# gaopinghai/BDE2VID

Measured on AMD Instinct MI355X. Metric: reconstructed frames/sec at 5x240x180 voxels, seq_len=16, higher is better.
Workload: dtype f32 (operands split into two fp16 terms on the matrix cores where conv_sb / lstm_sb / winblock_sb apply: 3 MFMAs per fp32 block, f32 accumulate)

## Files before the change

### bde2vid_amd/csrc/api_model.h

```cpp
#pragma once
namespace bde {

struct DenseLayer {
    int rows = 0, Cin = 0, KS = 1;
    std::vector<float> w, bias, lnsum;
};

struct PackedLayer {
    int Cin = 0, Cout = 0, KS = 1, CK = 8, nchunks = 0, ntiles = 0;
    bool lstm = false;
    long w_off = -1, b_off = -1, s_off = -1;
    long w_sz = 0;
    int G = 1;
    long sb_off = -1, sb_sz = 0;
    long sh_off = -1, sh_sz = 0;
    long sh_unscale_off = -1;
    long split_off(int terms) const { return terms == 2 ? sh_off : sb_off; }
    long split_sz(int terms) const { return terms == 2 ? sh_sz : sb_sz; }
    int sb_chunks = 0;
    long h3_off[2] = {-1, -1};
    long h3_sz[2] = {0, 0};
    mutable int sb_used = 0;
    int G_decide = 0;
};

static PackedLayer group_view(const PackedLayer& pl, int g) {
    PackedLayer v = pl;
    v.G_decide = pl.G;
    v.G = 1;
    v.w_off += g * pl.w_sz;
    if (v.b_off >= 0) v.b_off += (long)g * pl.Cout;
    if (v.s_off >= 0) v.s_off += (long)g * pl.Cout;
    if (v.sb_off >= 0) v.sb_off += g * pl.sb_sz;
    if (v.sh_off >= 0) v.sh_off += g * pl.sh_sz;
    return v;
}

struct Arena {
    std::vector<float> host;
    long alloc(long n) {
        long off = (long)host.size();
        long n4 = (n + 3) / 4 * 4;
        host.resize(off + n4, 0.f);
        return off;
    }
};

struct AttnBlock {
    PackedLayer qkv, proj, fc1, fc2;
    long proj16 = -1, fc1_16 = -1, fc2_16 = -1, qkv16 = -1;
    long projW = -1, fc1W = -1, fc2W = -1, qkvW = -1;
    long projS = -1, fc1S = -1, fc2S = -1, qkvS = -1;
    long projH = -1, fc1H = -1, fc2H = -1, qkvH = -1;
    long unscaleH = -1;
    long projHF = -1, projHF_unscale = -1;
    long fc1N = -1, fc2N = -1, mlpN_unscale = -1;
    long qkvN = -1, qkvN_unscale = -1;
    long kvpad_off = -1;
    long bias_off = -1;
    long biasF_off = -1;
    long biasW_off = -1;
};
struct AttnLevel {
    int depth = 0, C = 0;
    std::vector<AttnBlock> blocks;
    PackedLayer kvall;
    long kvallW = -1;
    long kvallH = -1, kvallH_unscale = -1;
};

struct Workspace {
    int T = 0, B = 0, H = 0, W = 0;
    std::vector<void*> allocs;
    float* ev = nullptr;
    float* head = nullptr;
    float* out = nullptr;
    std::vector<float*> xenc, gx, hseq, cst, merged, mergedT, kvun, kvref, dec, qkv0;
    float *qkv = nullptr, *ao = nullptr, *x1 = nullptr, *hid = nullptr, *xa = nullptr, *xb = nullptr;
    int* tile_count = nullptr;
    std::vector<float*> mergedS, mstats;
    float *xaS = nullptr, *xbS = nullptr, *stA = nullptr, *stB = nullptr;
    float* up = nullptr;
    float* sb = nullptr;
    float* sb2 = nullptr;
    long sb2_bytes = 0;
    std::vector<float*> gur, ghr, gou, gub;
    float *cat = nullptr, *fuse = nullptr;
    float *rbA = nullptr, *rbX[2] = {nullptr, nullptr}, *zero_l = nullptr;
    std::vector<float*> hsk;
    std::vector<float*> hsb, ghb;
    long sb_bytes = 0;
    hipGraphExec_t graph_exec = nullptr;
    int graph_part = 0;
    bool warm = false;
    void release() {
        if (graph_exec) { (void)hipGraphExecDestroy(graph_exec); graph_exec = nullptr; }
        warm = false;
        for (void* p : allocs) (void)hipFree(p);
        allocs.clear();
        ev = head = out = qkv = ao = x1 = hid = xa = xb = up = sb = sb2 = cat = fuse = rbA = rbX[0] = rbX[1] = zero_l = nullptr;
        tile_count = nullptr;
        xaS = xbS = stA = stB = nullptr;
        mergedS.clear(); mstats.clear();
        sb_bytes = sb2_bytes = 0;
        for (auto* v : {&xenc, &gx, &hseq, &cst, &merged, &mergedT, &kvun, &kvref, &dec, &qkv0, &gur, &ghr, &gou, &gub, &hsk, &hsb, &ghb}) v->clear();
        T = B = H = W = 0;
    }
};

}

using namespace bde;

struct bde_model {
    bde_config cfg;
    int L = 0;
    std::map<std::string, std::pair<std::vector<int64_t>, std::vector<float>>> raw;
    bool finalized = false;
    Arena arena;
    float* dev = nullptr;
    long dev_numel = 0;
    PackedLayer head, pred_dummy;
    std::vector<PackedLayer> enc, gx, lstm, lstm8, dec;
    std::vector<PackedLayer> lstm_sb;
    std::vector<PackedLayer> lstm_sbk;
    std::vector<PackedLayer> lstm_sbx;
    std::vector<PackedLayer> gru_ur, gru_o;
    std::vector<PackedLayer> dec_fuse;
    PackedLayer pred_fuse;
    std::vector<PackedLayer> rb1, rb2;
    std::vector<AttnLevel> attn;
    long predw_off = -1, predb_off = -1, zero_off = -1;
    static constexpr int MAX_SLOTS = 4;
    Workspace wslots[MAX_SLOTS];
    int cur = 0;
    Workspace& W() { return wslots[cur]; }
    hipStream_t cap_stream = nullptr;
    int use_graph = 1;
    int pipeline = 1;
    hipStream_t pstream[MAX_SLOTS] = {};
    hipEvent_t pin[MAX_SLOTS] = {}, pout[MAX_SLOTS] = {};
    bool pbusy[MAX_SLOTS] = {};
    hipStream_t last_stream = nullptr;
    long ncalls = 0;
    int device = 0;
    hipStream_t side[MAX_SLOTS + 1] = {};
    std::vector<hipEvent_t> frame_ev[MAX_SLOTS + 1];
    hipEvent_t join_ev[MAX_SLOTS + 1] = {};
    int overlap = 0;
    int eager_cut = 1;
    int overlap_chunk = 4;
    int debug_skip = 0;
    int tok_debug = 0;
    unsigned long long* tok_stamps = nullptr;
    Tuning tune;
    int lstm_hc8 = -1;
    int dir_mask = 3;
    int winblock = 1;
    int winblock_sb = 1;
    int fuse_pred = 1;
    int xcd_remap = 1;
    int head3 = 1;
    int fuse_enc_sb = 1;
    int conv_sb = 1;
    int sb_terms = BDE_DEFAULT_SB_TERMS;
    int lstm_two_streams = 0;
    hipStream_t dir_stream[4] = {};
    hipEvent_t dir_fork[4] = {}, dir_join[4] = {};
    int use_lstm_sbk = 1;
    int wide_kv_sb = 1;
    int wide_fuse_mlp = 1;
    int lstm_fuse_x = 1;
    int lstm_sb_mode = 0;
    long fused_min_tiles = 160;
    unsigned* ovf_dev = nullptr;
    unsigned* ovf_host = nullptr;
    int sb_auto = 1;
    long sb_overflows = 0;
    int sb_latched = 0;
    struct Pending {
        bool on = false;
        hipEvent_t done = nullptr;
        hipStream_t stream = nullptr;
        int T = 0, B = 0, H = 0, W = 0;
        std::vector<float*> images;
    } pend[MAX_SLOTS];
    unsigned* ovf() const { return (ovf_dev && sb_terms == 2) ? ovf_dev + cur : nullptr; }
    bool prof_on = false;
    struct ProfSpan { std::string name; hipEvent_t a, b; };
    std::vector<ProfSpan> prof;
    std::vector<hipEvent_t> prof_pool;

    int cin(int l) const { return cfg.basechannels << l; }
    int cout(int l) const { return cfg.basechannels << (l + 1); }
    const float* P(long off) const { return dev + off; }
    long lstm_sb_off(int l) const { return (size_t)l < lstm_sb.size() ? lstm_sb[l].sb_off : -1; }
    long zero_off_long() const { return zero_off; }
};

namespace bde {

static hipEvent_t prof_event(bde_model* m) {
    hipEvent_t e;
    if (!m->prof_pool.empty()) { e = m->prof_pool.back(); m->prof_pool.pop_back(); return e; }
    if (hipEventCreate(&e) != hipSuccess) return nullptr;
    return e;
}
struct ProfScope {
    bde_model* m; hipStream_t s; hipEvent_t a = nullptr, b = nullptr; const char* name;
    ProfScope(bde_model* m_, const char* n, hipStream_t s_) : m(m_), s(s_), name(n) {
        if (!m->prof_on) return;
        a = prof_event(m); b = prof_event(m);
        if (a) (void)hipEventRecord(a, s);
    }
    ~ProfScope() {
        if (!m->prof_on || !a || !b) return;
        (void)hipEventRecord(b, s);
        m->prof.push_back({name, a, b});
    }
};

static const char* pname(const char* base, int i) {
    static std::map<std::string, std::string> names;
    static std::mutex mu;
    const std::string k = std::string(base) + std::to_string(i);
// ... 6 lines not shown
```

### bde2vid_amd/csrc/api_schedule.h

```cpp
#pragma once
namespace bde {

struct ConvCall {
    const PackedLayer* pl = nullptr;
    const float* in = nullptr;
    float* out = nullptr;
    const float* res1 = nullptr;
    const float* res2 = nullptr;
    int N = 1, Hs = 0, Ws = 0;
    int stride = 1;
    int act = ACT_NONE;
    long in_gs = 0, out_gs = 0;
    int mask_w = 0, mask_pt = 0, mask_pl = 0;
    int cout_rows = -1;
    const float* pred_head = nullptr;
    float* pred_out = nullptr;
    float* out_sb = nullptr;
    long out_sb_gs = 0;
    bool in_sb = false;
    int decide_N = 0;
};

static bool conv_takes_sb(const bde_model* m, const PackedLayer& pl, int stride, int N, int Hs, int Ws) {
    const int pad = pl.KS / 2;
// ... 1051 lines not shown
}

static int run_bottleneck_level(bde_model* m, int l, int T, int B, int h, int w, hipStream_t s) {
    const bde_config& c = m->cfg;
    Workspace& ws = m->W();
    const int C = m->cout(l), nb = c.num_res_blocks;
    const long fs = (long)B * C * h * w;
    for (int t = 0; t < T; ++t) {
        ProfScope ps(m, pname("bottleneck", l), s);
        const int f = t + c.buffer_index[0];
        float* mt = ws.merged[l] + (long)t * fs;
        const float* x = (f < 0 || f >= T) ? ws.zero_l : ws.merged[l] + (long)f * fs;
        if (nb == 0) { BDE_TRY(add2(x, mt, mt, fs, s)); continue; }
        for (int k = 0; k < nb; ++k) {
            ConvCall c1;
            c1.pl = &m->rb1[k]; c1.in = x; c1.out = ws.rbA; c1.N = B; c1.Hs = h; c1.Ws = w; c1.act = ACT_RELU;
            BDE_TRY(run_conv(m, c1, s));
            const bool last = k == nb - 1;
            ConvCall c2;
            c2.pl = &m->rb2[k]; c2.in = ws.rbA; c2.N = B; c2.Hs = h; c2.Ws = w; c2.act = ACT_NONE;
            c2.res1 = x;
            c2.res2 = last ? mt : nullptr;
            c2.out = last ? mt : ws.rbX[k & 1];
            BDE_TRY(run_conv(m, c2, s));
            x = c2.out;
        }
    }
    return BDE_OK;
}

enum { PART_ALL = 0, PART_MAIN = 1, PART_TAIL = 2, PART_PRE = 3 };

static int run_decoder(bde_model* m, int j, const float* in, const float* skip, float* out, int N, int Hs, int Ws,
                       hipStream_t s, const float* pred_head = nullptr, float* pred_out = nullptr, int part = PART_ALL, int decide_N = 0) {
    const PackedLayer& pl = m->dec[j];
    Workspace& ws = m->W();
    if (decide_N <= 0) decide_N = N;
    const bool to_sb = m->fuse_enc_sb && (!pred_out || pl.Cout <= 32) && conv_takes_sb(m, pl, 1, decide_N, 2 * Hs, 2 * Ws) && ws.sb &&
                       split_bf16_bytes(N, pl.Cin, 4L * Hs * Ws) <= ws.sb_bytes;
    if (part != PART_TAIL) {
        ProfScope ps(m, pname("dec_up", j), s);
        if (to_sb) BDE_TRY(upsample2x_sum_split(in, skip, ws.sb, N, pl.Cin, Hs, Ws, m->sb_terms, m->ovf(), s));
        else BDE_TRY(upsample2x_sum(in, skip, ws.up, Hs, Ws, (long)N * pl.Cin, s));
    }
    if (part == PART_MAIN) return BDE_OK;
    ConvCall d;
    d.pl = &pl;
    d.in = to_sb ? ws.sb : ws.up;
    d.in_sb = to_sb;
    d.out = out;
    d.N = N;
    d.Hs = 2 * Hs;
    d.Ws = 2 * Ws;
    d.act = ACT_RELU6;
    d.pred_head = pred_head;
    d.pred_out = pred_out;
    d.decide_N = decide_N;
    ProfScope ps(m, pname("dec_conv", j), s);
    return run_conv(m, d, s);
}

static int check_dims(const bde_model* m, int T, int B, int H, int W) {
    const bde_config& c = m->cfg;
    BDE_REQUIRE(m->finalized, "weights are not finalized");
    BDE_REQUIRE(T >= 1 && B >= 1, "T=%d B=%d", T, B);
    const int mult = 1 << c.num_encoders;
    BDE_REQUIRE(H > 0 && W > 0 && H % mult == 0 && W % mult == 0, "H=%d W=%d must be multiples of %d", H, W, mult);
    for (int l = 0; l < c.num_encoders; ++l)
        if (c.depths[l] > 0)
            BDE_REQUIRE((H >> (l + 1)) >= 7 && (W >> (l + 1)) >= 7,
                        "feature map %dx%d at attention level %d is smaller than the 7x7 window (the reference "
                        "raises there too)", H >> (l + 1), W >> (l + 1), l);
    return BDE_OK;
}

static int forward_on(bde_model* m, const float* const* events, int T, int B, int H, int W, float* const* images,
                      hipStream_t s);

static int pipeline_stream(int slot, hipStream_t* out) {
    static hipStream_t pool[BDE_MAX_DEVICES][bde_model::MAX_SLOTS] = {};
    int d = 0;
    BDE_HIP(hipGetDevice(&d));
    BDE_REQUIRE(d >= 0 && d < BDE_MAX_DEVICES, "device %d", d);
    if (!pool[d][slot]) BDE_HIP(hipStreamCreateWithFlags(&pool[d][slot], hipStreamNonBlocking));
    *out = pool[d][slot];
    return BDE_OK;
}

static int note_overflow_readback(bde_model* m, hipStream_t s) {
    bde_model::Pending& p = m->pend[m->cur];
    if (!p.done) BDE_HIP(hipEventCreateWithFlags(&p.done, hipEventDisableTiming));
    BDE_HIP(hipMemcpyAsync(m->ovf_host + m->cur, m->ovf_dev + m->cur, sizeof(unsigned), hipMemcpyDeviceToHost, s));
    BDE_HIP(hipEventRecord(p.done, s));
    return BDE_OK;
}
static void note_pending(bde_model* m, int slot, hipStream_t s, int T, int B, int H, int W, float* const* images) {
    bde_model::Pending& p = m->pend[slot];
    p.on = true; p.stream = s; p.T = T; p.B = B; p.H = H; p.W = W;
    p.images.assign(images, images + T);
}
static int settle_overflow(bde_model* m) {
    bool flagged[bde_model::MAX_SLOTS] = {};
    int nflag = 0;
    for (int i = 0; i < bde_model::MAX_SLOTS; ++i) {
        bde_model::Pending& p = m->pend[i];
        if (!p.on) continue;
        BDE_HIP(hipEventSynchronize(p.done));
        if (m->ovf_host[i] != 0) { flagged[i] = true; ++nflag; }
    }
    if (nflag == 0) {
        for (auto& p : m->pend) p.on = false;
        return BDE_OK;
    }
    m->sb_overflows += nflag;
    for (int i = 0; i < bde_model::MAX_SLOTS; ++i) m->ovf_host[i] = 0;
    if (!m->sb_auto) {
        for (auto& p : m->pend) p.on = false;
        return fail(BDE_ERR_RANGE, "%d forward(s): an activation reached 65520, beyond the two fp16 terms of the default operand format "
                    "(csrc/split.h); the frames of those calls are not valid.  set_tuning(\"sb_terms\", 3) or \"sb_auto\" = 1", nflag);
    }
    for (int i = 0; i < bde_model::MAX_SLOTS; ++i)
        if (m->pend[i].on) BDE_HIP(hipStreamSynchronize(m->pend[i].stream));
    struct Redo { int slot; float* ev; long ev_fs; };
    std::vector<Redo> redo;
    for (int i = 0; i < bde_model::MAX_SLOTS; ++i) {
        if (!flagged[i]) continue;
        const bde_model::Pending& p = m->pend[i];
        const long ev_fs = (long)p.B * m->cfg.num_bins * p.H * p.W;
        float* ev = nullptr;
        BDE_HIP(hipMalloc((void**)&ev, sizeof(float) * ev_fs * p.T));
        BDE_HIP(hipMemcpy(ev, m->wslots[i].ev, sizeof(float) * ev_fs * p.T, hipMemcpyDeviceToDevice));
        redo.push_back({i, ev, ev_fs});
    }
    for (auto& w : m->wslots) w.release();
    m->sb_terms = 3;
    m->sb_latched = 1;
    int st = BDE_OK;
    for (const Redo& r : redo) {
        bde_model::Pending p = m->pend[r.slot];
        std::vector<const float*> evp(p.T);
        for (int t = 0; t < p.T; ++t) evp[t] = r.ev + (long)t * r.ev_fs;
        m->cur = r.slot;
        if (st == BDE_OK) st = forward_on(m, evp.data(), p.T, p.B, p.H, p.W, p.images.data(), p.stream);
        (void)hipStreamSynchronize(p.stream);
        (void)hipFree(r.ev);
    }
    m->cur = 0;
    for (auto& p : m->pend) p.on = false;
    return st;
}

static int forward_impl(bde_model* m, const float* const* events, int T, int B, int H, int W, float* const* images,
                        hipStream_t user) {
    if (m->pipeline < 2) {
        for (const auto& p : m->pend) if (p.on) { BDE_TRY(settle_overflow(m)); break; }
        m->cur = 0;
        BDE_TRY(forward_on(m, events, T, B, H, W, images, user));
        if (m->ovf() == nullptr) return BDE_OK;
        note_pending(m, 0, user, T, B, H, W, images);
        return settle_overflow(m);
    }
    const int slot = (int)(m->ncalls++ % m->pipeline);
    if (m->pend[slot].on) BDE_TRY(settle_overflow(m));
    if (!m->pstream[slot]) {
        BDE_TRY(pipeline_stream(slot, &m->pstream[slot]));
        BDE_HIP(hipEventCreateWithFlags(&m->pin[slot], hipEventDisableTiming));
        BDE_HIP(hipEventCreateWithFlags(&m->pout[slot], hipEventDisableTiming));
    }
    m->cur = slot;
    BDE_HIP(hipEventRecord(m->pin[slot], user));
    BDE_HIP(hipStreamWaitEvent(m->pstream[slot], m->pin[slot], 0));
    m->last_stream = m->pstream[slot];
    const int st = forward_on(m, events, T, B, H, W, images, m->pstream[slot]);
    if (st == BDE_OK && m->ovf() != nullptr) note_pending(m, slot, m->pstream[slot], T, B, H, W, images);
    BDE_HIP(hipEventRecord(m->pout[slot], m->pstream[slot]));
    m->pbusy[slot] = true;
    m->cur = 0;
    return st;
}

static int forward_body(bde_model* m, int T, int B, int H, int W, hipStream_t s, int part);
static bool side_decode_on(const bde_model* m, int T);

static int forward_on(bde_model* m, const float* const* events, int T, int B, int H, int W, float* const* images,
                      hipStream_t s) {
    BDE_TRY(check_dims(m, T, B, H, W));
    BDE_TRY(ensure_workspace(m, T, B, H, W));
    Workspace& ws = m->W();
    const long ev_fs = (long)B * m->cfg.num_bins * H * W, img_fs = (long)B * H * W;
    BDE_TRY(copy_frames(events, ws.ev, T, ev_fs, 0, s));
    ProfScope whole(m, "forward", s);
    const bool guard = m->ovf() != nullptr;
    const bool cut = guard && m->eager_cut && m->pipeline < 2 && m->fuse_enc_sb && !(m->debug_skip & (8 | 16)) && !m->prof_on;
    const int part_main = cut ? PART_MAIN : PART_ALL;
    if (guard) BDE_HIP(hipMemsetAsync(m->ovf(), 0, sizeof(unsigned), s));
    if (cut) BDE_TRY(forward_body(m, T, B, H, W, s, PART_PRE));
    const bool can_graph = m->use_graph && ws.warm && !side_decode_on(m, T);
    if (ws.graph_exec && ws.graph_part != part_main) { (void)hipGraphExecDestroy(ws.graph_exec); ws.graph_exec = nullptr; }
    if (can_graph && !ws.graph_exec) {
        if (!m->cap_stream) BDE_HIP(hipStreamCreateWithFlags(&m->cap_stream, hipStreamNonBlocking));
        hipGraph_t graph = nullptr;
        BDE_HIP(hipStreamBeginCapture(m->cap_stream, hipStreamCaptureModeRelaxed));
        const int st = forward_body(m, T, B, H, W, m->cap_stream, part_main);
        ws.graph_part = part_main;
        const hipError_t e = hipStreamEndCapture(m->cap_stream, &graph);
        hipError_t ei = hipSuccess;
        if (st == BDE_OK && e == hipSuccess) ei = hipGraphInstantiate(&ws.graph_exec, graph, nullptr, nullptr, 0);
        if (graph) (void)hipGraphDestroy(graph);
        if (st != BDE_OK || e != hipSuccess || ei != hipSuccess) {
            (void)hipGetLastError();
            ws.graph_exec = nullptr;
            m->use_graph = 0;
        }
    }
    if (m->use_graph && can_graph && ws.graph_exec) {
        BDE_HIP(hipGraphLaunch(ws.graph_exec, s));
    } else {
        BDE_TRY(forward_body(m, T, B, H, W, s, part_main));
        ws.warm = true;
    }
    if (guard && cut) BDE_TRY(note_overflow_readback(m, s));
    if (cut) BDE_TRY(forward_body(m, T, B, H, W, s, PART_TAIL));
    if (guard && !cut) BDE_TRY(note_overflow_readback(m, s));
    BDE_TRY(copy_frames(images, ws.out, T, img_fs, 1, s));
    return BDE_OK;
}

static int decode_frames(bde_model* mm, int f0, int nf, int T_, int B_, int H_, int W_, hipStream_t st, int part = PART_ALL) {
    Workspace& w = mm->W();
    const int L_ = mm->L;
    const float* x = w.merged[L_ - 1] + (long)f0 * mm->cout(L_ - 1) * (H_ >> L_) * (W_ >> L_);
    for (int j = 0; j < L_; ++j) {
        const int l = L_ - 1 - j;
        const long in_fs = (long)mm->cout(l) * (H_ >> (l + 1)) * (W_ >> (l + 1));
        const long out_fs = (long)mm->cin(l) * (H_ >> l) * (W_ >> l);
        const bool lastj = j == L_ - 1;
        const int jpart = part == PART_ALL ? PART_ALL : (lastj ? part : (part == PART_MAIN ? PART_ALL : -1));
        if (jpart >= 0) {
            ProfScope ps(mm, "decoder", st);
            const bool fuse = lastj && pred_fusable(mm);
            const float* skip = w.merged[l] + (long)f0 * in_fs;
            if (mm->cfg.skip_concat) {
                if (jpart != PART_TAIL)
                    BDE_TRY(run_concat_fuse(mm, mm->dec_fuse[j], skip, x, nf, mm->cout(l), (long)(H_ >> (l + 1)) * (W_ >> (l + 1)), st));
                x = w.fuse;
                skip = nullptr;
            }
            BDE_TRY(run_decoder(mm, j, x, skip, w.dec[j] + (long)f0 * out_fs, nf,
                                H_ >> (l + 1), W_ >> (l + 1), st,
                                fuse ? w.head + (long)f0 * mm->cfg.basechannels * H_ * W_ : nullptr,
                                fuse ? w.out + (long)f0 * H_ * W_ : nullptr, jpart, T_ * B_));
        }
        x = w.dec[j] + (long)f0 * out_fs;
    }
    if (part == PART_MAIN) return BDE_OK;
    if (pred_fusable(mm)) return BDE_OK;
    const long total = (long)nf * H_ * W_;
    long blocks = std::min<long>(cdivl(total, 256), 4096);
    ProfScope ps(mm, "pred", st);
    const float* hd = w.head + (long)f0 * mm->cfg.basechannels * H_ * W_;
    if (mm->cfg.skip_concat) {
        BDE_TRY(run_concat_fuse(mm, mm->pred_fuse, x, hd, nf, mm->cfg.basechannels, (long)H_ * W_, st));
        x = w.fuse;
        hd = nullptr;
    }
    hipLaunchKernelGGL(pred_kernel, dim3((unsigned)blocks), dim3(256), 0, st, x,
                       hd, mm->P(mm->predw_off),
                       mm->P(mm->predb_off), w.out + (long)f0 * H_ * W_, mm->cfg.basechannels, (long)H_ * W_, total,
                       mm->cfg.activation);
    BDE_HIP(hipGetLastError());
    return BDE_OK;
}

static bool side_decode_on(const bde_model* m, int T) {
    const bde_config& c = m->cfg;
    const bool plain_flags = c.use_rc && c.recurrent_type == 0 && !c.skip_concat && c.depths[c.num_encoders - 1] > 0;
    return m->overlap != 0 && plain_flags && !(m->debug_skip & (2 | 8)) && !m->prof_on && T > m->overlap_chunk;
}

static int forward_body(bde_model* m, int T, int B, int H, int W, hipStream_t s, int part) {
    const bde_config& c = m->cfg;
    Workspace& ws = m->W();
    const int L = c.num_encoders;
    const long TB = (long)T * B;
    const bool side_decode = side_decode_on(m, T);
    const int last_chunk_t0 = side_decode ? (T - 1) / m->overlap_chunk * m->overlap_chunk : 0;
    const int tail_f0 = last_chunk_t0 * B, tail_nf = (int)TB - tail_f0;
    if (part == PART_TAIL) return (m->debug_skip & 8) ? BDE_OK : decode_frames(m, tail_f0, tail_nf, T, B, H, W, s, PART_TAIL);
    if (part != PART_MAIN) {
        { ProfScope ps(m, "head", s); BDE_TRY(run_head_conv(m, ws.ev, ws.head, (int)TB, H, W, s)); }
        if (!(m->debug_skip & 16)) BDE_TRY(run_enc_gx(m, 0, ws.head, 0, (int)TB, T, B, H, W, s));
        if (part == PART_PRE) return BDE_OK;
    }
    struct SideCtx { int T, B, H, W, chunk, slot; hipStream_t main, side; };
    static auto decode_fn = decode_frames;
    const int slot = (m->cap_stream && s == m->cap_stream) ? bde_model::MAX_SLOTS : m->cur;
    if (side_decode && !m->side[slot]) {
        int lo = 0, hi = 0;
        BDE_HIP(hipDeviceGetStreamPriorityRange(&lo, &hi));
        BDE_HIP(hipStreamCreateWithPriority(&m->side[slot], hipStreamNonBlocking, lo));
        BDE_HIP(hipEventCreateWithFlags(&m->join_ev[slot], hipEventDisableTiming));
    }
    while (side_decode && (int)m->frame_ev[slot].size() < T) {
        hipEvent_t e;
        BDE_HIP(hipEventCreateWithFlags(&e, hipEventDisableTiming));
        m->frame_ev[slot].push_back(e);
    }
    const float* target = ws.head;
    bool decoded = false;
    for (int l = 0; l < L; ++l) {
        const int Hl = H >> l, Wl = W >> l, h = Hl / 2, w = Wl / 2, C = m->cout(l);
        BDE_TRY(run_recurrent_level(m, l, target, T, B, Hl, Wl, s, l == 0));
        const long n = TB * C * h * w;
        { ProfScope ps(m, pname("merge", l), s); BDE_TRY(add2(ws.hseq[l], ws.hseq[l] + n, ws.merged[l], n, s)); }
        if (c.depths[l] > 0 && !(m->debug_skip & (l == 0 ? 1 : 2))) {
            static const char* names[BDE_MAX_LEVELS] = {"attn0", "attn1", "attn2", "attn3", "attn4", "attn5", "attn6", "attn7"};
            ProfScope ps(m, names[l], s);
            SideCtx sc{T, B, H, W, m->overlap_chunk, slot, s, m->side[slot]};
            FrameDoneFn fn = nullptr;
            const bool fork = side_decode && l == L - 1;
            if (fork) {
                fn = [](bde_model* mm, int t, void* vp) -> int {
                    SideCtx* q = (SideCtx*)vp;
                    const int done = t + 1;
                    if (done % q->chunk != 0 || done > (q->T - 1) / q->chunk * q->chunk) return BDE_OK;
                    const int t0 = done - q->chunk;
                    BDE_HIP(hipEventRecord(mm->frame_ev[q->slot][t], q->main));
                    BDE_HIP(hipStreamWaitEvent(q->side, mm->frame_ev[q->slot][t], 0));
                    return decode_fn(mm, t0 * q->B, q->chunk * q->B, q->T, q->B, q->H, q->W, q->side, PART_ALL);
                };
            }
            BDE_TRY(run_attention_level(m, l, T, B, h, w, s, fn, &sc));
            if (fork) {
                BDE_HIP(hipEventRecord(m->join_ev[slot], m->side[slot]));
                BDE_HIP(hipStreamWaitEvent(s, m->join_ev[slot], 0));
                decoded = true;
            }
        }
        if (l == L - 1 && c.depths[l] == 0) BDE_TRY(run_bottleneck_level(m, l, T, B, h, w, s));
        target = ws.merged[l];
    }
    if (m->debug_skip & 8) return BDE_OK;
    const int dpart = part == PART_MAIN ? PART_MAIN : PART_ALL;
    if (decoded) return decode_frames(m, tail_f0, tail_nf, T, B, H, W, s, dpart);
    return decode_frames(m, 0, (int)TB, T, B, H, W, s, dpart);
}

static int validate_config(const bde_config* c) {
    BDE_REQUIRE(c != nullptr, "null config");
    BDE_REQUIRE(c->num_encoders >= 1 && c->num_encoders <= BDE_MAX_LEVELS, "num_encoders=%d", c->num_encoders);
    BDE_REQUIRE(c->num_bins >= 1 && c->basechannels >= 1, "num_bins=%d basechannels=%d", c->num_bins, c->basechannels);
    BDE_REQUIRE(c->ks == 3 || c->ks == 5, "ks=%d (3 or 5)", c->ks);
    BDE_REQUIRE(c->frame_num >= 1 && c->frame_num <= BDE_MAX_FRAMES, "frame_num=%d", c->frame_num);
    BDE_REQUIRE(c->q_idx >= 0 && c->q_idx < c->frame_num, "q_idx=%d", c->q_idx);
    BDE_REQUIRE(c->buffer_index[c->q_idx] == 0, "buffer_index[q_idx] must be 0 (the query frame is the current frame)");
    BDE_REQUIRE(c->activation == 0 || c->activation == 1, "activation=%d", c->activation);
    BDE_REQUIRE(c->recurrent_type == 0 || c->recurrent_type == 1, "recurrent_type=%d (0 ConvLSTM, 1 ConvGRU)", c->recurrent_type);
    BDE_REQUIRE(c->use_rc == 0 || c->use_rc == 1, "use_rc=%d", c->use_rc);
    BDE_REQUIRE(c->skip_concat == 0 || c->skip_concat == 1, "skip_concat=%d", c->skip_concat);
    BDE_REQUIRE(c->norm >= 0 && c->norm <= 2, "norm=%d (0 none, 1 BN, 2 IN)", c->norm);
    BDE_REQUIRE(c->num_res_blocks >= 0 && c->num_res_blocks <= 64, "num_res_blocks=%d", c->num_res_blocks);
    for (int l = 0; l < c->num_encoders; ++l) {
        BDE_REQUIRE(c->depths[l] >= 0, "depths[%d]=%d", l, c->depths[l]);
        if (c->depths[l] > 0) {
            const int C = c->basechannels << (l + 1);
            BDE_REQUIRE(c->num_heads >= 1 && C % c->num_heads == 0, "C=%d not divisible by %d heads", C, c->num_heads);
            const int hd = C / c->num_heads;
            BDE_REQUIRE(hd == 1 || hd == 2 || hd == 4 || hd == 8 || hd == 16 || hd == 32, "head_dim=%d not built", hd);
        }
    }
    return BDE_OK;
}


}
```

### bde2vid_amd/csrc/bde_api.hip

```cpp
#include <hip/hip_runtime.h>

#include <algorithm>
#include <cmath>
#include <cstdlib>
#include <map>
#include <memory>
#include <mutex>
#include <string>
#include <vector>

#include "../../include/bde2vid.h"
#include "attn.h"
#include "common.h"
#include "conv_mfma.h"
#include "pw_gemm.h"
#include "token_fused.h"
#include "lstm16.h"
#include "lstm_sb.h"
#include "winblock.h"
#include "winblock_sb.h"
#include "wideblock.h"
#include "wide_mlp.h"
#include "wide_core.h"
#include "conv_vec.h"
#include "conv_sb.h"
#include "voxel.h"
#include "metrics.h"

namespace bde {

int conv_tu_occupancy(const char* kernel);

std::string& last_error_ref() {
    static thread_local std::string e;
    return e;
}
int fail(int code, const char* fmt, ...) {
    char buf[1024];
    va_list ap;
    va_start(ap, fmt);
    vsnprintf(buf, sizeof buf, fmt, ap);
    va_end(ap);
    last_error_ref() = buf;
    return code;
}
}

#include "api_elementwise.h"
#include "api_model.h"
#include "api_pack.h"
#include "api_schedule.h"


extern "C" {
#pragma GCC visibility push(default)

const char* bde_last_error(void) { return last_error_ref().c_str(); }
int bde_abi_version(void) { return 4; }

int bde_create(const bde_config* cfg, bde_model** out) {
    BDE_REQUIRE(out != nullptr, "null out");
    BDE_TRY(validate_config(cfg));
    bde_model* m = new bde_model();
    if (const char* e = getenv("BDE_SB_TERMS")) {
        if (e[0] == '3' && e[1] == 0) m->sb_terms = 3;
        else if (e[0] == '2' && e[1] == 0) m->sb_terms = 2;
    }
    m->cfg = *cfg;
    m->L = cfg->num_encoders;
    *out = m;
    return BDE_OK;
}

void bde_destroy(bde_model* m) {
    if (!m) return;
    for (auto& w : m->wslots) w.release();
    if (m->cap_stream) (void)hipStreamDestroy(m->cap_stream);
    for (int i = 0; i < bde_model::MAX_SLOTS; ++i) {
        if (m->pin[i]) (void)hipEventDestroy(m->pin[i]);
        if (m->pout[i]) (void)hipEventDestroy(m->pout[i]);
    }
    if (m->dev) (void)hipFree(m->dev);
    if (m->ovf_dev) (void)hipFree(m->ovf_dev);
    if (m->ovf_host) (void)hipHostFree(m->ovf_host);
    for (auto& p : m->pend) if (p.done) (void)hipEventDestroy(p.done);
    for (int i = 0; i < 4; ++i) {
        if (m->dir_fork[i]) (void)hipEventDestroy(m->dir_fork[i]);
        if (m->dir_join[i]) (void)hipEventDestroy(m->dir_join[i]);
        if (m->dir_stream[i]) (void)hipStreamDestroy(m->dir_stream[i]);
    }
    for (auto& sp : m->prof) { (void)hipEventDestroy(sp.a); (void)hipEventDestroy(sp.b); }
    for (auto e : m->prof_pool) (void)hipEventDestroy(e);
    for (int i = 0; i <= bde_model::MAX_SLOTS; ++i) {
        for (auto e : m->frame_ev[i]) (void)hipEventDestroy(e);
        if (m->join_ev[i]) (void)hipEventDestroy(m->join_ev[i]);
        if (m->side[i]) (void)hipStreamDestroy(m->side[i]);
    }
    delete m;
}

int bde_load_weight(bde_model* m, const char* key, const float* data, const int64_t* shape, int32_t ndim) {
    BDE_REQUIRE(m && key && data && shape && ndim >= 1 && ndim <= 8, "bad argument");
    int64_t n = 1;
    std::vector<int64_t> sh(shape, shape + ndim);
    for (auto v : sh) {
        BDE_REQUIRE(v >= 1, "weight '%s' has a non-positive dimension", key);
        n *= v;
    }
    m->raw[key] = {sh, std::vector<float>(data, data + n)};
    m->finalized = false;
    return BDE_OK;
}

int bde_finalize_weights(bde_model* m) {
    BDE_REQUIRE(m != nullptr, "null model");
    BDE_TRY(build_packed(m));
    BDE_HIP(hipGetDevice(&m->device));
    return upload(m);
}

int bde_alloc_packed(bde_model* m) {
    BDE_REQUIRE(m != nullptr, "null model");
    const bde_config& c = m->cfg;
    auto put = [&](const std::string& k, std::vector<int64_t> sh) {
        int64_t n = 1;
        for (auto v : sh) n *= v;
        m->raw[GP + k] = {sh, std::vector<float>((size_t)n, 0.f)};
    };
    const int L = c.num_encoders, ks = c.ks, bc = c.basechannels;
    auto put_convlayer = [&](const std::string& p, int cout, int cin) {
        put(p + "conv2d.weight", {cout, cin, ks, ks});
        if (c.norm != 1) put(p + "conv2d.bias", {cout});
        if (c.norm == 1) { put(p + "norm_layer.weight", {cout}); put(p + "norm_layer.bias", {cout}); }
        if (c.norm) { put(p + "norm_layer.running_mean", {cout}); put(p + "norm_layer.running_var", {cout}); }
    };
    put_convlayer("head.", bc, c.num_bins);
    const char* dirs[2] = {"forward_encoder", "backward_encoder"};
    for (int d = 0; d < 2; ++d)
        for (int l = 0; l < L; ++l) {
            std::string p = std::string(dirs[d]) + "." + std::to_string(l) + ".";
            const int ci = bc << l, co = bc << (l + 1);
            if (!c.use_rc) { put_convlayer(p, co, ci); continue; }
            put_convlayer(p + "conv.", co, ci);
            if (c.recurrent_type == 1) {
                for (const char* gate : {"update_gate", "reset_gate", "out_gate"}) {
                    put(p + "recurrent_block." + gate + ".weight", {co, 2 * co, 3, 3});
                    put(p + "recurrent_block." + gate + ".bias", {co});
                }
            } else {
                put(p + "recurrent_block.Gates.weight", {4 * co, 2 * co, 3, 3});
                put(p + "recurrent_block.Gates.bias", {4 * co});
            }
        }
    if (c.depths[L - 1] == 0)
        for (int k = 0; k < c.num_res_blocks; ++k) {
            std::string p = "feat_attns." + std::to_string(L - 1) + "." + std::to_string(1 + k) + ".";
            const int C = bc << L;
            put(p + "conv1.weight", {C, C, 3, 3}); put(p + "conv1.bias", {C});
            put(p + "conv2.weight", {C, C, 3, 3}); put(p + "conv2.bias", {C});
        }
    const int tbl = (2 * c.frame_num - 1) * 169;
    for (int l = 0; l < L; ++l) {
        const int C = bc << (l + 1);
// ... 62 lines not shown
    TuningScope ts(&m->tune);
    int T, B, H, W;
    m->cur = 0;
    BDE_TRY(split_dims(m, &T, &B, &H, &W));
    Workspace& ws = m->W();
    const float* target = level == 0 ? ws.head : ws.merged[level - 1];
    m->dir_mask = 1 << direction;
    const int st = run_recurrent_level(m, level, target, T, B, H >> level, W >> level, (hipStream_t)stream);
    m->dir_mask = 3;
    return st;
}

int bde_split_attend(bde_model* m, int32_t level, void* stream) {
    BDE_REQUIRE(m && level >= 0 && level < m->L, "bad argument");
    TuningScope ts(&m->tune);
    hipStream_t s = (hipStream_t)stream;
    int T, B, H, W;
    m->cur = 0;
    BDE_TRY(split_dims(m, &T, &B, &H, &W));
    Workspace& ws = m->W();
    const int h = H >> (level + 1), w = W >> (level + 1);
    const long n = (long)T * B * m->cout(level) * h * w;
    BDE_TRY(add2(ws.hseq[level], ws.hseq[level] + n, ws.merged[level], n, s));
    if (m->cfg.depths[level] > 0) return run_attention_level(m, level, T, B, h, w, s);
    if (level == m->L - 1) return run_bottleneck_level(m, level, T, B, h, w, s);
    return BDE_OK;
}

int bde_split_decode(bde_model* m, float* const* images, void* stream) {
    BDE_REQUIRE(m && images, "null argument");
    TuningScope ts(&m->tune);
    hipStream_t s = (hipStream_t)stream;
    int T, B, H, W;
    m->cur = 0;
    BDE_TRY(split_dims(m, &T, &B, &H, &W));
    for (int t = 0; t < T; ++t) BDE_REQUIRE(images[t], "null frame pointer at t=%d", t);
    BDE_TRY(decode_frames(m, 0, T * B, T, B, H, W, s));
    BDE_TRY(copy_frames(images, m->W().out, T, (long)B * H * W, 1, s));
    if (m->ovf()) {
        unsigned v = 0;
        BDE_HIP(hipMemcpyAsync(m->ovf_host, m->ovf(), sizeof v, hipMemcpyDeviceToHost, s));
        BDE_HIP(hipStreamSynchronize(s));
        v = m->ovf_host[0];
        m->ovf_host[0] = 0;
        if (v) {
            BDE_HIP(hipMemset(m->ovf(), 0, sizeof v));
            ++m->sb_overflows;
            return fail(BDE_ERR_RANGE, "split forward: an activation reached 65520, beyond the two fp16 terms of the default operand "
                        "format (csrc/split.h); set_tuning(\"sb_terms\", 3) on both ranks and run it again");
        }
    }
    return BDE_OK;
}

int bde_split_buffer(bde_model* m, const char* what, int32_t level, int32_t direction, float** ptr, int64_t* numel) {
    BDE_REQUIRE(m && what && ptr && numel && level >= 0 && level < m->L, "bad argument");
    int T, B, H, W;
    m->cur = 0;
    BDE_TRY(split_dims(m, &T, &B, &H, &W));
    Workspace& ws = m->W();
    const long n = (long)T * B * m->cout(level) * (long)(H >> (level + 1)) * (W >> (level + 1));
    const std::string k(what);
    if (k == "hidden") {
        BDE_REQUIRE(direction == 0 || direction == 1, "direction=%d", direction);
        *ptr = ws.hseq[level] + (long)direction * n;
    } else if (k == "level_out") {
        *ptr = ws.merged[level];
    } else {
        return fail(BDE_ERR_ARG, "unknown split buffer '%s' (hidden | level_out)", what);
    }
    *numel = n;
    return BDE_OK;
}

int bde_wait_outputs(bde_model* m, void* stream) {
    BDE_REQUIRE(m != nullptr, "null model");
    TuningScope ts(&m->tune);
    const int st = settle_overflow(m);
    for (int i = 0; i < bde_model::MAX_SLOTS; ++i)
        if (m->pbusy[i]) {
            BDE_HIP(hipStreamWaitEvent((hipStream_t)stream, m->pout[i], 0));
            m->pbusy[i] = false;
        }
    return st;
}

int bde_set_tuning(bde_model* m, const char* key, int64_t value) {
    BDE_REQUIRE(m && key, "null argument");
    if (std::string(key) == "graph") { m->use_graph = (int)value; return BDE_OK; }
    if (std::string(key) == "pipeline") {
        BDE_REQUIRE(value >= 1 && value <= bde_model::MAX_SLOTS, "pipeline depth must be 1..%d", bde_model::MAX_SLOTS);
        m->pipeline = (int)value;
        return BDE_OK;
    }
    if (std::string(key) == "sb_auto") {
        BDE_REQUIRE(value == 0 || value == 1, "sb_auto: 0 (an overflow of the two-term format fails the call) or 1 (recompute with three terms)");
        m->sb_auto = (int)value;
        return BDE_OK;
    }
    {
        TuningScope ts(&m->tune);
        for (const auto& p : m->pend) if (p.on) { BDE_TRY(settle_overflow(m)); break; }
    }
    for (auto& w : m->wslots)
        if (w.graph_exec) { (void)hipGraphExecDestroy(w.graph_exec); w.graph_exec = nullptr; }
    if (std::string(key) == "lstm_hc8") { m->lstm_hc8 = (int)value; return BDE_OK; }
    if (std::string(key) == "winblock") {
        if (m->winblock != (int)value)
            for (auto& w : m->wslots) w.release();
        m->winblock = (int)value;
        return BDE_OK;
    }
    if (std::string(key) == "winblock_sb") { m->winblock_sb = (int)value; return BDE_OK; }
    if (std::string(key) == "wide_kv_sb" || std::string(key) == "wide_fuse_mlp") {
        int& v = std::string(key) == "wide_kv_sb" ? m->wide_kv_sb : m->wide_fuse_mlp;
        if (v != (int)value)
            for (auto& w : m->wslots) w.release();
        v = (int)value;
        return BDE_OK;
    }
    if (std::string(key) == "conv_sb") {
        if (m->conv_sb != (int)value)
            for (auto& w : m->wslots) w.release();
        m->conv_sb = (int)value;
        return BDE_OK;
    }
    if (std::string(key) == "sb_terms") {
        BDE_REQUIRE(value == 2 || value == 3, "sb_terms: 2 (two fp16 terms) or 3 (three bf16 terms)");
        if (m->sb_terms != (int)value)
            for (auto& w : m->wslots) w.release();
        m->sb_terms = (int)value;
        m->sb_latched = 0;
        return BDE_OK;
    }
    if (std::string(key) == "fuse_enc_sb") { m->fuse_enc_sb = (int)value; return BDE_OK; }
    if (std::string(key) == "head3") { m->head3 = (int)value; return BDE_OK; }
    if (std::string(key) == "xcd_remap") { m->xcd_remap = (int)value; return BDE_OK; }
    if (std::string(key) == "lstm_two_streams") { m->lstm_two_streams = (int)value; return BDE_OK; }
    if (std::string(key) == "lstm_fuse_x") {
        if (m->lstm_fuse_x != (int)value)
            for (auto& w : m->wslots) w.release();
        m->lstm_fuse_x = (int)value;
        return BDE_OK;
    }
    if (std::string(key) == "lstm_sbk") {
        if (m->use_lstm_sbk != (int)value)
            for (auto& w : m->wslots) w.release();
        m->use_lstm_sbk = (int)value;
        return BDE_OK;
    }
    if (std::string(key) == "lstm_sb") {
        if (m->lstm_sb_mode != (int)value)
            for (auto& w : m->wslots) w.release();
        m->lstm_sb_mode = (int)value;
        return BDE_OK;
    }
    if (std::string(key) == "fuse_pred") { m->fuse_pred = (int)value; return BDE_OK; }
    if (std::string(key) == "fused_min_tiles") { m->fused_min_tiles = value; return BDE_OK; }
    if (std::string(key) == "pw_batched") { m->tune.pw_batched = (int)value; return BDE_OK; }
    if (std::string(key) == "pw_force") { m->tune.pw_force = (int)value; return BDE_OK; }
    if (std::string(key) == "conv_nt") { m->tune.conv_nt = (int)value; return BDE_OK; }
    if (std::string(key) == "conv_vec") { m->tune.conv_vec = (int)value; return BDE_OK; }
    if (std::string(key) == "lstm_shape") { m->tune.lstm_shape = (int)value; return BDE_OK; }
    if (std::string(key) == "tok_npt") { m->tune.tok_npt = (int)value; return BDE_OK; }
    if (std::string(key) == "tok_debug") { m->tok_debug = (int)value; return BDE_OK; }
    if (std::string(key) == "overlap") { m->overlap = (int)value; return BDE_OK; }
    if (std::string(key) == "eager_cut") { m->eager_cut = (int)value; return BDE_OK; }
    if (std::string(key) == "debug_skip") { m->debug_skip = (int)value; return BDE_OK; }
    if (std::string(key) == "overlap_chunk") { m->overlap_chunk = std::max<int>(1, (int)value); return BDE_OK; }
    return fail(BDE_ERR_ARG, "unknown tuning key '%s'", key);
}

int bde_get_info(const bde_model* m, const char* key, int64_t* value) {
    BDE_REQUIRE(m && key && value, "null argument");
    const std::string k(key);
    if (k == "debug_skip") *value = m->debug_skip;
    else if (k == "graph") *value = m->use_graph;
    else if (k == "graphs_live") {
        int64_t n = 0;
        for (const auto& w : m->wslots) n += w.graph_exec != nullptr;
        *value = n;
    } else if (k == "pipeline") *value = m->pipeline;
    else if (k == "last_stream") *value = (int64_t)(uintptr_t)m->last_stream;
    else if (k == "device") *value = m->device;
    else if (k == "winblock") *value = m->winblock;
    else if (k == "winblock_sb") *value = m->winblock_sb;
    else if (k == "conv_sb") *value = m->conv_sb;
    else if (k == "head3") *value = m->head3;
    else if (k == "lstm_sb") *value = m->lstm_sb_mode;
    else if (k == "lstm_sbk") *value = m->use_lstm_sbk;
    else if (k == "lstm_fuse_x") *value = m->lstm_fuse_x;
    else if (k == "wide_kv_sb") *value = m->wide_kv_sb;
    else if (k == "wide_fuse_mlp") *value = m->wide_fuse_mlp;
    else if (k == "wide_core2") {
        int64_t v = 0;
        for (int l = 0; l < m->L; ++l) v |= wide_ok(m, l) && split_chain_ok(m, l);
        *value = v;
    }
    else if (k == "sb_terms") *value = m->sb_terms;
    else if (k == "sb_auto") *value = m->sb_auto;
    else if (k == "sb_overflows") *value = m->sb_overflows;
    else if (k == "sb_latched") *value = m->sb_latched;
    else if (k == "sb_overflow_word") {
        unsigned v = 0;
        if (m->ovf_dev) {
            BDE_HIP(hipDeviceSynchronize());
            BDE_HIP(hipMemcpy(&v, m->ovf_dev, sizeof v, hipMemcpyDeviceToHost));
            BDE_HIP(hipMemset(m->ovf_dev, 0, sizeof v));
        }
        *value = v;
    }
    else if (k == "packed_numel") *value = m->dev_numel;
    else if (k == "sb_head") *value = m->head.sb_used;
    else if (k.compare(0, 3, "sb_") == 0 && k.size() >= 5 && k.back() >= '0' && k.back() - '0' < m->L) {
        const int i = k.back() - '0';
        const std::string what = k.substr(3, k.size() - 4);
        if (what == "enc") *value = m->enc[i].sb_used;
        else if (what == "gx") *value = m->gx[i].sb_used;
        else if (what == "dec") *value = m->dec[i].sb_used;
        else if (what == "lstm") *value = (size_t)i < m->lstm_sbk.size() ? m->lstm_sbk[i].sb_used : 0;
        else return fail(BDE_ERR_ARG, "unknown info key '%s'", key);
    }
    else return fail(BDE_ERR_ARG, "unknown info key '%s'", key);
    return BDE_OK;
}

int bde_debug_token_stamps(bde_model* m, int64_t* host_out, int32_t n) {
    BDE_REQUIRE(m != nullptr, "null model");
    if (!m->tok_stamps) {
        BDE_HIP(hipMalloc((void**)&m->tok_stamps, sizeof(unsigned long long) * 64 * 4 * 8));
        BDE_HIP(hipMemset(m->tok_stamps, 0, sizeof(unsigned long long) * 64 * 4 * 8));
        BDE_HIP(hipMemset(m->tok_stamps + 2046, 0xff, sizeof(unsigned long long)));
    }
    if (host_out) {
        BDE_HIP(hipDeviceSynchronize());
        BDE_HIP(hipMemcpy(host_out, m->tok_stamps, sizeof(int64_t) * std::min(n, 64 * 4 * 8), hipMemcpyDeviceToHost));
        BDE_HIP(hipMemset(m->tok_stamps + 2046, 0xff, sizeof(unsigned long long)));
        BDE_HIP(hipMemset(m->tok_stamps + 2047, 0, sizeof(unsigned long long)));
    }
    return BDE_OK;
}

int bde_debug_conv_shape(int32_t ks, int32_t stride, int32_t cout, int32_t in_h, int32_t in_w, int32_t* row_tiles) {
    const int pad = ks / 2;
    const int Ho = (in_h + 2 * pad - ks) / stride + 1, Wo = (in_w + 2 * pad - ks) / stride + 1;
    const int terms = BDE_DEFAULT_SB_TERMS;
    const int shape = conv_sb_pick(ks, stride, cout, in_w, Ho, Wo, terms);
    if (row_tiles) {
        if (shape == SB_32x256T) *row_tiles = -conv_sb_tile_cols(256, Ho, Wo);
        else if (shape == SB_64x128T) *row_tiles = -conv_sb_tile_cols(128, Ho, Wo);
        else *row_tiles = shape == SB_NONE ? 0 : conv_sb_tile_mode(ks, stride, shape == SB_128x64 ? 64 : 128, in_w, Ho, Wo, terms);
    }
    return shape;
}

float bde_debug_split(const float* x, int64_t n, int32_t terms, float scale, uint16_t* out) {
    if (!x || !out || n <= 0 || (terms != 2 && terms != 3)) return 0.f;
    for (int64_t i = 0; i < n; ++i) {
        unsigned short t[3];
        split_terms(x[i], terms, scale, t);
        for (int k = 0; k < terms; ++k) out[i * terms + k] = t[k];
    }
    return terms == 2 ? sb_weight_scale(x, (long)n) : 1.f;
}

// ... 325 lines not shown
```

Measured before the change: 1931.

## Stagger pipelined slots with lead events and stream priorities

Adds a stagger point: each pipelined call records an event partway through the level loop (default after level 0's attention), and the next slot's stream waits on it. Consecutive frames then start offset rather than all contending at once. Odd pipeline slots get created with a different stream priority, and overflow settling now waits only on the slot being reused instead of all pending work. The intent is to reduce contention between concurrent slots while still overlapping them; the cost is added cross-stream dependencies that could serialize work, and graphs are rebuilt when the stagger point changes.

```diff
diff --git a/bde2vid_amd/csrc/api_model.h b/bde2vid_amd/csrc/api_model.h
--- a/bde2vid_amd/csrc/api_model.h
+++ b/bde2vid_amd/csrc/api_model.h
@@ -92,6 +92,7 @@
     long sb_bytes = 0;
     hipGraphExec_t graph_exec = nullptr;
     int graph_part = 0;
+    int graph_lead = 0;
     bool warm = false;
     void release() {
         if (graph_exec) { (void)hipGraphExecDestroy(graph_exec); graph_exec = nullptr; }
@@ -141,6 +142,9 @@
     hipStream_t pstream[MAX_SLOTS] = {};
     hipEvent_t pin[MAX_SLOTS] = {}, pout[MAX_SLOTS] = {};
     bool pbusy[MAX_SLOTS] = {};
+    int stagger = 2;
+    hipEvent_t lead[MAX_SLOTS] = {};
+    int lead_from = -1;
     hipStream_t last_stream = nullptr;
     long ncalls = 0;
     int device = 0;
diff --git a/bde2vid_amd/csrc/api_schedule.h b/bde2vid_amd/csrc/api_schedule.h
--- a/bde2vid_amd/csrc/api_schedule.h
+++ b/bde2vid_amd/csrc/api_schedule.h
@@ -1157,7 +1157,15 @@
     int d = 0;
     BDE_HIP(hipGetDevice(&d));
     BDE_REQUIRE(d >= 0 && d < BDE_MAX_DEVICES, "device %d", d);
-    if (!pool[d][slot]) BDE_HIP(hipStreamCreateWithFlags(&pool[d][slot], hipStreamNonBlocking));
+    if (!pool[d][slot]) {
+        if (slot & 1) {
+            int lo = 0, hi = 0;
+            BDE_HIP(hipDeviceGetStreamPriorityRange(&lo, &hi));
+            BDE_HIP(hipStreamCreateWithPriority(&pool[d][slot], hipStreamNonBlocking, lo));
+        } else {
+            BDE_HIP(hipStreamCreateWithFlags(&pool[d][slot], hipStreamNonBlocking));
+        }
+    }
     *out = pool[d][slot];
     return BDE_OK;
 }
@@ -1225,28 +1233,43 @@
     return st;
 }
 
+static int settle_slot(bde_model* m, int slot) {
+    bde_model::Pending& p = m->pend[slot];
+    if (!p.on) return BDE_OK;
+    BDE_HIP(hipEventSynchronize(p.done));
+    if (m->ovf_host[slot] != 0) return settle_overflow(m);
+    p.on = false;
+    return BDE_OK;
+}
+
+static int lead_point(const bde_model* m) { return m->pipeline >= 2 ? m->stagger : 0; }
+
 static int forward_impl(bde_model* m, const float* const* events, int T, int B, int H, int W, float* const* images,
                         hipStream_t user) {
     if (m->pipeline < 2) {
         for (const auto& p : m->pend) if (p.on) { BDE_TRY(settle_overflow(m)); break; }
         m->cur = 0;
+        m->lead_from = -1;
         BDE_TRY(forward_on(m, events, T, B, H, W, images, user));
         if (m->ovf() == nullptr) return BDE_OK;
         note_pending(m, 0, user, T, B, H, W, images);
         return settle_overflow(m);
     }
     const int slot = (int)(m->ncalls++ % m->pipeline);
-    if (m->pend[slot].on) BDE_TRY(settle_overflow(m));
+    BDE_TRY(settle_slot(m, slot));
     if (!m->pstream[slot]) {
         BDE_TRY(pipeline_stream(slot, &m->pstream[slot]));
         BDE_HIP(hipEventCreateWithFlags(&m->pin[slot], hipEventDisableTiming));
         BDE_HIP(hipEventCreateWithFlags(&m->pout[slot], hipEventDisableTiming));
+        BDE_HIP(hipEventCreateWithFlags(&m->lead[slot], hipEventDisableTiming));
     }
     m->cur = slot;
     BDE_HIP(hipEventRecord(m->pin[slot], user));
     BDE_HIP(hipStreamWaitEvent(m->pstream[slot], m->pin[slot], 0));
+    if (m->lead_from >= 0 && m->lead_from != slot) BDE_HIP(hipStreamWaitEvent(m->pstream[slot], m->lead[m->lead_from], 0));
     m->last_stream = m->pstream[slot];
     const int st = forward_on(m, events, T, B, H, W, images, m->pstream[slot]);
+    m->lead_from = (st == BDE_OK && lead_point(m) > 0) ? slot : -1;
     if (st == BDE_OK && m->ovf() != nullptr) note_pending(m, slot, m->pstream[slot], T, B, H, W, images);
     BDE_HIP(hipEventRecord(m->pout[slot], m->pstream[slot]));
     m->pbusy[slot] = true;
@@ -1271,13 +1294,17 @@
     if (guard) BDE_HIP(hipMemsetAsync(m->ovf(), 0, sizeof(unsigned), s));
     if (cut) BDE_TRY(forward_body(m, T, B, H, W, s, PART_PRE));
     const bool can_graph = m->use_graph && ws.warm && !side_decode_on(m, T);
-    if (ws.graph_exec && ws.graph_part != part_main) { (void)hipGraphExecDestroy(ws.graph_exec); ws.graph_exec = nullptr; }
+    if (ws.graph_exec && (ws.graph_part != part_main || ws.graph_lead != lead_point(m))) {
+        (void)hipGraphExecDestroy(ws.graph_exec);
+        ws.graph_exec = nullptr;
+    }
     if (can_graph && !ws.graph_exec) {
         if (!m->cap_stream) BDE_HIP(hipStreamCreateWithFlags(&m->cap_stream, hipStreamNonBlocking));
         hipGraph_t graph = nullptr;
         BDE_HIP(hipStreamBeginCapture(m->cap_stream, hipStreamCaptureModeRelaxed));
         const int st = forward_body(m, T, B, H, W, m->cap_stream, part_main);
         ws.graph_part = part_main;
+        ws.graph_lead = lead_point(m);
         const hipError_t e = hipStreamEndCapture(m->cap_stream, &graph);
         hipError_t ei = hipSuccess;
         if (st == BDE_OK && e == hipSuccess) ei = hipGraphInstantiate(&ws.graph_exec, graph, nullptr, nullptr, 0);
@@ -1383,11 +1410,17 @@
     }
     const float* target = ws.head;
     bool decoded = false;
+    const int lead_at = lead_point(m);
+    auto mark_lead = [&](int point) -> int {
+        if (point == lead_at && m->lead[m->cur]) BDE_HIP(hipEventRecord(m->lead[m->cur], s));
+        return BDE_OK;
+    };
     for (int l = 0; l < L; ++l) {
         const int Hl = H >> l, Wl = W >> l, h = Hl / 2, w = Wl / 2, C = m->cout(l);
         BDE_TRY(run_recurrent_level(m, l, target, T, B, Hl, Wl, s, l == 0));
         const long n = TB * C * h * w;
         { ProfScope ps(m, pname("merge", l), s); BDE_TRY(add2(ws.hseq[l], ws.hseq[l] + n, ws.merged[l], n, s)); }
+        BDE_TRY(mark_lead(2 * l + 1));
         if (c.depths[l] > 0 && !(m->debug_skip & (l == 0 ? 1 : 2))) {
             static const char* names[BDE_MAX_LEVELS] = {"attn0", "attn1", "attn2", "attn3", "attn4", "attn5", "attn6", "attn7"};
             ProfScope ps(m, names[l], s);
@@ -1413,6 +1446,7 @@
             }
         }
         if (l == L - 1 && c.depths[l] == 0) BDE_TRY(run_bottleneck_level(m, l, T, B, h, w, s));
+        BDE_TRY(mark_lead(2 * l + 2));
         target = ws.merged[l];
     }
     if (m->debug_skip & 8) return BDE_OK;
diff --git a/bde2vid_amd/csrc/bde_api.hip b/bde2vid_amd/csrc/bde_api.hip
--- a/bde2vid_amd/csrc/bde_api.hip
+++ b/bde2vid_amd/csrc/bde_api.hip
@@ -79,6 +79,7 @@
     for (int i = 0; i < bde_model::MAX_SLOTS; ++i) {
         if (m->pin[i]) (void)hipEventDestroy(m->pin[i]);
         if (m->pout[i]) (void)hipEventDestroy(m->pout[i]);
+        if (m->lead[i]) (void)hipEventDestroy(m->lead[i]);
     }
     if (m->dev) (void)hipFree(m->dev);
     if (m->ovf_dev) (void)hipFree(m->ovf_dev);
@@ -307,6 +308,7 @@
             BDE_HIP(hipStreamWaitEvent((hipStream_t)stream, m->pout[i], 0));
             m->pbusy[i] = false;
         }
+    m->lead_from = -1;
     return st;
 }
 
@@ -329,6 +331,12 @@
     }
     for (auto& w : m->wslots)
         if (w.graph_exec) { (void)hipGraphExecDestroy(w.graph_exec); w.graph_exec = nullptr; }
+    if (std::string(key) == "stagger") {
+        BDE_REQUIRE(value >= 0 && value <= 2 * m->L, "stagger: 0 (off) or the stage boundary 1..%d (2l+1: behind level l's recurrent "
+                    "steps, 2l+2: behind its attention block)", 2 * m->L);
+        m->stagger = (int)value;
+        return BDE_OK;
+    }
     if (std::string(key) == "lstm_hc8") { m->lstm_hc8 = (int)value; return BDE_OK; }
     if (std::string(key) == "winblock") {
         if (m->winblock != (int)value)
@@ -406,6 +414,12 @@
         for (const auto& w : m->wslots) n += w.graph_exec != nullptr;
         *value = n;
     } else if (k == "pipeline") *value = m->pipeline;
+    else if (k == "stagger") *value = m->stagger;
+    else if (k == "pending_slots") {
+        int64_t n = 0;
+        for (const auto& p : m->pend) n += p.on;
+        *value = n;
+    }
     else if (k == "last_stream") *value = (int64_t)(uintptr_t)m->last_stream;
     else if (k == "device") *value = m->device;
     else if (k == "winblock") *value = m->winblock;
```

New measurement: 2356 (median of 6 runs). 1.22x the previous value.
